# thomasjacumin/optical-flow-optimal-transport

Hardware: AMD Instinct MI355X
Metric: BB solver iters/sec on 640×480×32 grid (higher is better)
Workload: dtype f64; 1 GPU; FOTO Benamou-Brenier outer iteration, 640x480x32, r=1, eps=1e-2, CG rtol=1e-6 (scipy rule), stop rules off; cg_mode=spectral-gauss, parallelism=single GPU

## Files before the change

optical-flow-optimal-transport_amd/csrc/foto_bb.cpp:

```cpp
#include <rccl/rccl.h>

#include <algorithm>
#include <chrono>
#include <cmath>
#include <cstddef>
#include <cstring>
#include <memory>
#include <utility>

#include "foto_devmem.h"
#include "foto_internal.h"
#include "foto_spectral.h"
#include "foto_xfer.h"

namespace foto {

#define FOTO_NCCL_CHECK(call)                                                                 \
    do {                                                                                     \
        ncclResult_t r_ = (call);                                                            \
        if (r_ != ncclSuccess) {                                                             \
            ::foto::set_error("%s:%d %s: %s", __FILE__, __LINE__, #call, ncclGetErrorString(r_)); \
            return FOTO_ERR_COMM;                                                            \
        }                                                                                    \
    } while (0)
// ... 227 lines not shown
    hipStream_t user = nullptr;
};

static int load_rho(foto_bb_ctx* c, Shard& s, const RhoSrc& src) {
    const int64_t nxy = (int64_t)c->Nx * c->Ny;
    if (!src.i0) {
        FOTO_HIP_CHECK(hipMemcpyAsync(s.rho0, src.h0, nxy * sizeof(double), hipMemcpyHostToDevice, c->s));
        FOTO_HIP_CHECK(hipMemcpyAsync(s.rhoT, src.hT, nxy * sizeof(double), hipMemcpyHostToDevice, c->s));
        return 0;
    }
    if (!c->sh.empty() && c->sh[0].get() != &s) {
        FOTO_HIP_CHECK(hipMemcpyAsync(s.rho0, c->sh[0]->rho0, nxy * sizeof(double), hipMemcpyDeviceToDevice, c->s));
        FOTO_HIP_CHECK(hipMemcpyAsync(s.rhoT, c->sh[0]->rhoT, nxy * sizeof(double), hipMemcpyDeviceToDevice, c->s));
        return 0;
    }
    FOTO_TRY(c->link.enter(src.user, c->s));
    FOTO_HIP_CHECK(launch_ingest(*src.i0, c->Nx, c->Ny, s.rho0, c->s));
    FOTO_HIP_CHECK(launch_ingest(*src.iT, c->Nx, c->Ny, s.rhoT, c->s));
    if (src.normalize) {
        if (!c->nrm) {
            FOTO_TRY(s.alloc(sizeof(double) * (2 + (size_t)capped_blocks(nxy, SUM_MAX_BLOCKS)), &c->nrm));
        }
        double* const rho[2] = {s.rho0, s.rhoT};
        for (int k = 0; k < 2; ++k) {
            FOTO_HIP_CHECK(launch_sum(nxy, rho[k], c->nrm + 2, c->nrm + k, c->s));
            FOTO_HIP_CHECK(launch_div_scalar(nxy, rho[k], c->nrm + k, c->s));
        }
        FOTO_HIP_CHECK(hipMemcpyAsync(c->hsum, c->nrm, 2 * sizeof(double), hipMemcpyDeviceToHost, c->s));
    }
    return 0;
}

static int init_fields(foto_bb_ctx* c, Shard& s, const RhoSrc& src) {
    FOTO_TRY(load_rho(c, s, src));
    FOTO_HIP_CHECK(launch_init_mu(s.g, s.rho0, s.rhoT, s.mu[0], s.mu[1], s.mu[2], s.q[0], s.q[1], s.q[2], c->s));
    return 0;
}

static RhoSrc dev_src(const foto_image* f0, const foto_image* f1, int normalize, void* stream) {
    RhoSrc src;
    src.i0 = f0;
    src.iT = f1;
    src.normalize = normalize != 0;
    src.user = (hipStream_t)stream;
    return src;
}
static int dev_src_done(foto_bb_ctx* c, const RhoSrc& src, double* sums2_or_null) {
    FOTO_TRY(c->link.leave(c->s, src.user));
    if (sums2_or_null) {
        sums2_or_null[0] = src.normalize ? c->hsum[0] : 1.0;
        sums2_or_null[1] = src.normalize ? c->hsum[1] : 1.0;
    }
    return 0;
}

static int ctx_init(foto_bb_ctx* c, const RhoSrc& src) {
    const int64_t nxy = (int64_t)c->Nx * c->Ny;
    if (c->o.device >= 0) FOTO_HIP_CHECK(hipSetDevice(c->o.device));
    FOTO_TRY(stream_acquire(&c->s));
    FOTO_HIP_CHECK(hipHostMalloc((void**)&c->hS, sizeof(CGScal)));
    const int W = c->W;
    for (int k = 0; k < 2; ++k) {
        FOTO_HIP_CHECK(hipHostMalloc((void**)&c->hgath[k], sizeof(double) * 4 * W,
                                     hipHostMallocMapped | hipHostMallocCoherent));
        FOTO_HIP_CHECK(hipHostGetDevicePointer((void**)&c->dgath[k], c->hgath[k], 0));
    }
    for (auto& p : c->ph)
        for (int k = 0; k < 4; ++k)
            FOTO_HIP_CHECK(hipEventCreateWithFlags(&p[k], k < 3 ? hipEventDisableSystemFence : hipEventDefault));
    for (auto& e : c->fl) FOTO_HIP_CHECK(hipEventCreate(&e));
    if (c->rccl) {
        ncclUniqueId id;
        memcpy(&id, c->o.nccl_id, sizeof(id));
        FOTO_NCCL_CHECK(ncclCommInitRank(&c->nc, W, id, c->o.rank));
        if (c->tn.comm_stream) {
            FOTO_TRY(stream_acquire(&c->sc));
            FOTO_HIP_CHECK(hipEventCreateWithFlags(&c->cfork, hipEventDisableTiming));
            FOTO_HIP_CHECK(hipEventCreateWithFlags(&c->cjoin, hipEventDisableTiming));
            for (auto& e : c->cpart) FOTO_HIP_CHECK(hipEventCreateWithFlags(&e, hipEventDisableTiming));
        }
    }
    const int nlocal = c->rccl ? 1 : W;
    {
        c->fuse = c->tn.fuse_pr;
        c->pipe = W == 1 && c->fuse && c->o.cg_mode == 3 && c->tn.pipe;
        c->phase_force = c->tn.phase_ev;
        c->hcrit = W == 1 && c->fuse && c->tn.host_crit;
        const unsigned ff = c->hcrit ? hipEventDisableSystemFence : 0u;
        for (auto& e : c->fin) FOTO_HIP_CHECK(hipEventCreateWithFlags(&e, hipEventDisableTiming | ff));
    }
    for (int j = 0; j < nlocal; ++j) {
        auto sp = std::make_unique<Shard>();
        Shard& s = *sp;
        s.rank = c->rccl ? c->o.rank : j;
        s.g.Nt = c->Nt; s.g.Ny = c->Ny; s.g.Nx = c->Nx; s.g.nxy = nxy;
        if (split_planes(c->Nt, W, s.rank, &s.g.t0, &s.g.nloc) != 0) {
            set_error("world size %d exceeds Nt = %d (each rank needs >= 1 time slab)", W, c->Nt);
            return FOTO_ERR_ARG;
        }
        for (int f = 0; f < 3; ++f) { FOTO_TRY(s.alloc_field(&s.mu[f], c->s)); FOTO_TRY(s.alloc_field(&s.q[f], c->s)); }
        if (c->fuse)
            for (int f = 0; f < 3; ++f) FOTO_TRY(s.alloc_field(&s.nu[f], c->s));
        if (c->pipe) {
            for (int f = 0; f < 3; ++f) FOTO_TRY(s.alloc_field(&s.xi[f], c->s));
            FOTO_TRY(s.alloc_field(&s.phi_alt, c->s, 2));
        }
        if (c->fuse && W > 1) {
            FOTO_TRY(s.alloc_field(&s.wt, c->s));
            FOTO_TRY(s.alloc_zeroed(sizeof(double) * 8 * nxy, &s.edge, c->s));
        }
        FOTO_TRY(s.alloc_field(&s.phi, c->s, 2));
        FOTO_TRY(s.alloc_field(&s.rv, c->s));
        FOTO_TRY(s.alloc_field(&s.p[0], c->s));
        FOTO_TRY(s.alloc_field(&s.p[1], c->s));
        for (double** plane : {&s.rho0, &s.rhoT, &s.px, &s.py, &s.fu, &s.fv, &s.fm})
            FOTO_TRY(s.alloc(nxy * sizeof(double), plane));
        const int64_t nb = std::max<int64_t>(march_blocks(s.g), flat_blocks((int64_t)s.g.nloc * nxy));
        s.rb.cap = (int)std::max<int64_t>(2 * nb, 3 * (int64_t)prox_rhs_blocks(s.g, c->tn.pr_tch));
        FOTO_TRY(s.alloc(sizeof(double) * s.rb.cap, &s.rb.partials));
        FOTO_TRY(s.alloc_zeroed(sizeof(unsigned) * 64, &s.rb.ticket, c->s));
        FOTO_TRY(s.alloc_zeroed(sizeof(double) * 4 * W, &s.gath, c->s));
        FOTO_TRY(s.alloc_zeroed(sizeof(CGScal), &s.S, c->s));
        FOTO_TRY(init_fields(c, s, src));
        if (c->o.cg_mode >= 1 && c->o.cg_mode <= 3) {
            s.spec.reset(new SpectralPlan());
            FOTO_TRY(s.spec->init(s.g, s.rank, W, c->r, c->eps, c->o.cg_mode, c->tn, c->s));
        }
        c->sh.push_back(std::move(sp));
    }
    if (c->pipe && !(c->sh[0]->spec && c->sh[0]->spec->gauss())) c->pipe = false;
    FOTO_HIP_CHECK(hipStreamSynchronize(c->s));
    return 0;
}


static CGArgs cg_args(foto_bb_ctx* c, const Shard& s) {
    CGArgs a;
    a.r = c->r;
    a.eps = c->eps;
    a.rtol = c->o.cg_rtol;
    a.world = c->W;
    a.rank = s.rank;
    return a;
}

static int cg_iteration(foto_bb_ctx* c, int k) {
    const int W = c->W;
    const bool fused = (W == 1);
    if (!fused)
        for (auto& sp : c->sh) {
            Shard& s = *sp;
            FOTO_HIP_CHECK(launch_cg_pupd(s.g, k, s.rv, s.p[k & 1], s.p[(k + 1) & 1], s.S, s.gath_rr(), cg_args(c, s),
                                          c->s));
        }
    if (!fused) FOTO_TRY(halo(c, [k](Shard& s) { return s.p[(k + 1) & 1]; }));
    for (auto& sp : c->sh) {
        Shard& s = *sp;
        const CGArgs a = cg_args(c, s);
        const double nv = (double)s.g.nloc * (double)s.g.nxy;
        hipEvent_t e = c->kt.start(c->s);
        FOTO_HIP_CHECK(launch_cg_dir(s.g, k, s.rv, s.p[k & 1], s.p[(k + 1) & 1], a, s.S, s.rb, s.gath_rr(),
                                     s.gath_pap(W), fused ? 1 : 0, c->s));
        c->kt.stop(e, c->s, FOTO_K_CG_DIR, fused ? (k == 0 ? 16.0 : 24.0) * nv : 8.0 * nv);
    }
    FOTO_TRY(allgather(c, [W](Shard& s) { return s.gath_pap(W); }, 1));
    for (auto& sp : c->sh) {
        Shard& s = *sp;
// ... 1398 lines not shown
```

optical-flow-optimal-transport_amd/csrc/foto_internal.h:

```cpp
#pragma once

#include <hip/hip_runtime.h>

#include <algorithm>
#include <cstdint>
#include <cstdlib>
#include <cstdio>
#include <string>
#include <vector>

#include "../../include/foto.h"
#include "foto_tuning.h"

namespace foto {

void set_error(const char* fmt, ...);

#define FOTO_HIP_CHECK(call)                                                                  \
    do {                                                                                     \
        hipError_t e_ = (call);                                                              \
        if (e_ != hipSuccess) {                                                              \
            ::foto::set_error("%s:%d %s: %s", __FILE__, __LINE__, #call, hipGetErrorString(e_)); \
            return FOTO_ERR_HIP;                                                             \
        }                                                                                    \
// ... 117 lines not shown
    size_t count_before(size_t m) const {
        size_t n = 0;
        while (n < pend.size() && pend[n].id < m) ++n;
        return n;
    }
    void discard_from(size_t m) {
        const size_t keep = count_before(m);
        for (size_t k = keep; k < pend.size(); ++k) {
            pool.push_back(pend[k].a);
            pool.push_back(pend[k].b);
        }
        pend.resize(keep);
    }
    void resolve_upto(size_t m) { resolve_first(count_before(m)); }
    void resolve_first(size_t n) {
        n = std::min(n, pend.size());
        for (size_t k = 0; k < n; ++k) {
            Pend& p = pend[k];
            float t = 0.f;
            if (hipEventElapsedTime(&t, p.a, p.b) == hipSuccess) {
                this->n[p.cls] += 1;
                ms[p.cls] += t;
                bytes[p.cls] += p.bytes;
            }
            pool.push_back(p.a);
            pool.push_back(p.b);
        }
        pend.erase(pend.begin(), pend.begin() + n);
    }
    void resolve() { resolve_first(pend.size()); }
    void reset() {
        std::fill(n, n + 8, 0);
        std::fill(ms, ms + 8, 0.0);
        std::fill(bytes, bytes + 8, 0.0);
    }
    ~KTimer() {
        for (auto& p : pend) { (void)hipEventDestroy(p.a); (void)hipEventDestroy(p.b); }
        for (auto e : pool) (void)hipEventDestroy(e);
    }
};


struct CGArgs {
    double r, eps, rtol;
    int world, rank;
};

hipError_t launch_apply_A(const Geo& g, const double* p, double* out, double r, double eps, int lap_only,
                          hipStream_t s);
hipError_t launch_grad_st(const Geo& g, const double* phi, double* gt, double* gx, double* gy, hipStream_t s);
hipError_t launch_div_st(const Geo& g, const double* wt, const double* wx, const double* wy, double* out,
                         hipStream_t s);
hipError_t launch_grad2(int Nx, int Ny, const double* f, double* gx, double* gy, int bcD, hipStream_t s);
hipError_t launch_div2(int Nx, int Ny, const double* u, const double* v, double* out, int bcD, double sign,
                       hipStream_t s);
hipError_t launch_grad2_forward(int Nx, int Ny, const double* f, double* gx, double* gy, hipStream_t s);
hipError_t launch_stepB(int64_t M, const double* pa, const double* p1, const double* p2, double* qa,
                        double* q1, double* q2, hipStream_t s);
hipError_t launch_init_mu(const Geo& g, const double* rho0, const double* rhoT, double* mut, double* mux,
                          double* muy, double* qt, double* qx, double* qy, hipStream_t s);
hipError_t launch_rhs(const Geo& g, const double* mut, const double* mux, const double* muy, const double* qt,
                      const double* qx, const double* qy, const double* rho0, const double* rhoT, double r,
                      double* F, RedBuf rb, double* gath, int rank, hipStream_t s);
constexpr int REPORT_PIECE = 2048;
inline int report_pieces(int64_t nxy) { return (int)((nxy + REPORT_PIECE - 1) / REPORT_PIECE); }
struct ReportIn {
    const double *rho, *m1, *m2, *phi;
    const double *rho_lo, *rho_hi, *phi_lo, *phi_hi;
    const double *rho0, *rhoT;
};
hipError_t launch_report(const Geo& g, const ReportIn& in, double* part, unsigned* ticket, double* out,
                         hipStream_t s);
hipError_t launch_cg_dir(const Geo& g, int k, const double* rvec, const double* pold, double* pnew,
                         const CGArgs& a, CGScal* S, RedBuf rb, const double* gath_rr, double* gath_pap,
                         int fused, hipStream_t s);
hipError_t launch_cg_pupd(const Geo& g, int k, const double* rvec, const double* pold, double* pnew,
                          CGScal* S, const double* gath_rr, const CGArgs& a, hipStream_t s);
hipError_t launch_cg_upd(const Geo& g, int k, const double* p, double* x, double* rvec, const CGArgs& a,
                         CGScal* S, RedBuf rb, const double* gath_pap, double* gath_rr, hipStream_t s);
hipError_t launch_prox(const Geo& g, const double* phi, double* mut, double* mux, double* muy, double* qt,
                       double* qx, double* qy, double r, RedBuf rb, double* gath, int rank, hipStream_t s,
                       const int* guard = nullptr);
int prox_rhs_blocks(const Geo& g, int tch);
hipError_t launch_prox_rhs(const Geo& g, const double* phi, const double* mut, const double* mux, const double* muy,
                           double* nut, double* nux, double* nuy, const double* rho0, const double* rhoT, double r,
                           double* F, RedBuf rb, double* gath_crit, double* gath_rr, int tch, hipStream_t s,
                           const int* guard = nullptr, int defer_lo = 0, int defer_hi = 0, double* wt_out = nullptr,
                           double* edge = nullptr, double* hcrit = nullptr, int wt_pre = 0);
hipError_t launch_wt_pre(const Geo& g, const double* phi, const double* mut, const double* mux, const double* muy,
                         double r, double* wt, int defer_lo, int defer_hi, hipStream_t s, const int* guard = nullptr);
hipError_t launch_rhs_edge(const Geo& g, int n, const double* wt, const double* edge, const double* rho0,
                           const double* rhoT, double r, double* F, RedBuf rb, double* gath_rr, hipStream_t s,
                           const int* guard = nullptr);
hipError_t launch_q_from_phi(const Geo& g, const double* phi, const double* mut, const double* mux,
                             const double* muy, double* qt, double* qx, double* qy, double r, hipStream_t s);
hipError_t launch_traj(const Geo& g, const double* phi, int n_lo, int n_hi, double* px, double* py,
                       int init, hipStream_t s);
hipError_t launch_flow_record(int Nx, int Ny, const double* px, const double* py, void* ou, void* ov, void* om,
                              int dtype, int layout, hipStream_t s);

hipError_t launch_track(const Geo& g, const double* phi, int n_lo, int n_hi, const void* pts, int pts_dtype,
                        const double* pos_in, double* pos_out, void* out, int dtype, int64_t M, int all_steps,
                        hipStream_t s);

hipError_t launch_dot_self(int64_t n, const double* x, RedBuf rb, double* gath, int rank, hipStream_t s);

hipError_t launch_gn_coeffs(int w, int h, const double* f1, const double* f2, double* fx, double* fy,
                            double* ft, hipStream_t s);
hipError_t launch_gn_rhs(int w, int h, const double* fx, const double* fy, const double* f2, const double* ft,
                         double* b, hipStream_t s);
hipError_t launch_gn_apply(int w, int h, const double* fx, const double* fy, const double* f2, double alpha,
                           double lam, const double* x, double* y, hipStream_t s);
int gn_bj_solve(const double* f1, const double* f2, int w, int h, double alpha, double lam, double rtol, int maxiter,
                double* u, double* v, double* m, int* iterations);

int image_check(const foto_image* im, int w, int h, const char* who);
int image_dev_check(const foto_image* im, int w, int h, int device, const char* who);
int dev_ptr_check(const void* p, size_t bytes, int device, const char* who, const char* what);
int export_check(const void* out, int dtype, int layout, int64_t n, int device, const char* who);
int track_arg_check(const void* pts, const void* out, int64_t M, int all_steps, const char* who);
int track_dtype_check(const void* p, int dtype, const char* who, const char* what);
hipError_t launch_ingest(const foto_image& im, int w, int h, double* dst, hipStream_t s);
hipError_t launch_sum(int64_t n, const double* x, double* part, double* tot, hipStream_t s);
hipError_t launch_div_scalar(int64_t n, double* x, const double* S, hipStream_t s);
hipError_t launch_export(int64_t n, const double* a, const double* b, const double* c, void* out, int dtype,
                         int layout, hipStream_t s);
constexpr int FRAMES_MAX = 128;
struct FrameArgs {
    const double* a[FRAMES_MAX];
    const double* b[FRAMES_MAX];
    double w[FRAMES_MAX];
};
hipError_t launch_frames(const FrameArgs& fa, int count, int64_t n, double scale, void* out, int dtype,
                         hipStream_t s);

constexpr int MAPS_MAX = 128;
constexpr int MT_W = 32, MT_H = 8;
constexpr int PLANE_SEGS = 32;
struct MapTimes {
    double s[MAPS_MAX];
};
struct PlaneSegs {
    const double* base[PLANE_SEGS];
    int t0[PLANE_SEGS], nloc[PLANE_SEGS];
    int n;
};
hipError_t launch_plane_table(const PlaneSegs& sg, int64_t nxy, const double** table, hipStream_t s);
hipError_t launch_maps(const double* const* table, int Nt, int Nx, int Ny, const double* s, int count, int inv_iters,
                       void* out, int dtype, hipStream_t st);
hipError_t launch_interp(const double* const* table, int Nt, int Nx, int Ny, const foto_image& f0, int64_t sc0,
                         const foto_image& f1, int64_t sc1, int channels, const double* s, int count, int inv_iters,
                         void* out, int out_dtype, hipStream_t st);
int maps_arg_check(const double* s, const void* out, int count, int inv_iters, int Nt, const char* who);
int interp_frame_check(const foto_image* f, int channels, int64_t stride_c, int w, int h, const char* who);
size_t interp_frame_bytes(const foto_image* f, int channels, int64_t stride_c, int w, int h);
int flow_check(const foto_flow* fl, int w, int h, const char* who);
size_t flow_bytes(const foto_flow* fl, int w, int h);
inline bool overlaps(const void* a, size_t na, const void* b, size_t nb) {
    const uintptr_t a0 = (uintptr_t)a, b0 = (uintptr_t)b;
    return a0 < b0 + nb && b0 < a0 + na;
}

struct DevScratch {
    void* p = nullptr;
    size_t cap = 0;
    int reserve(size_t bytes, hipStream_t s) {
// ... 20 lines not shown
```

optical-flow-optimal-transport_amd/csrc/foto_kernels.hip:

```cpp
#include "foto_devutil.h"
#include "foto_internal.h"
#include "foto_reduce.h"

namespace foto {


__device__ __forceinline__ double row_A(const Geo& g, int t, int y, int x, double c, double xm, double xp,
                                        double ym, double yp, double tm, double tp, double r, double reps) {
    const bool ht = t > 0, hT = t < g.Nt - 1, hy = y > 0, hY = y < g.Ny - 1, hx = x > 0, hX = x < g.Nx - 1;
    const double cnt = (double)((int)ht + (int)hT + (int)hy + (int)hY + (int)hx + (int)hX);
    const double mr = -r;
    const double dg = r * cnt + reps;
    double s = 0.0;
    if (ht) s += mr * tm;
    if (hy) s += mr * ym;
    if (hx) s += mr * xm;
    s += dg * c;
    if (hX) s += mr * xp;
    if (hY) s += mr * yp;
    if (hT) s += mr * tp;
    return s;
}

__device__ __forceinline__ double row_L(const Geo& g, int t, int y, int x, double c, double xm, double xp,
                                        double ym, double yp, double tm, double tp) {
    const bool ht = t > 0, hT = t < g.Nt - 1, hy = y > 0, hY = y < g.Ny - 1, hx = x > 0, hX = x < g.Nx - 1;
    const double cnt = (double)((int)ht + (int)hT + (int)hy + (int)hY + (int)hx + (int)hX);
    double s = 0.0;
    if (ht) s += tm;
    if (hy) s += ym;
    if (hx) s += xm;
    s += (-cnt) * c;
    if (hX) s += xp;
    if (hY) s += yp;
    if (hT) s += tp;
    return s;
}

__device__ __forceinline__ int xcd_tile(int b) {
    constexpr int NXCD = 8;
    const int nb = gridDim.x, per = nb / NXCD, rem = nb % NXCD;
    const int xcd = b % NXCD, local = b / NXCD;
    return xcd * per + min(xcd, rem) + local;
}

template <class Val, class Body>
__device__ __forceinline__ void march(const Geo& g, int tile_blk, Val val, Body body) {
    const int tile = xcd_tile(tile_blk);
    constexpr int LW = TX + 2, LP = (TY + 2) * LW;
    __shared__ double lds[2 * LP];
    const int ntx = (g.Nx + TX - 1) / TX;
    const int x0 = (tile % ntx) * TX, y0 = (tile / ntx) * TY;
    const int tid = threadIdx.x, tx = tid & (TX - 1), ty = tid / TX;
    const int x = x0 + tx, y = y0 + ty;
    const bool in = (x < g.Nx) && (y < g.Ny);
    const int64_t off = in ? (int64_t)y * g.Nx + x : 0;
    int hx = -1, hy = -1, hl = -1;
    if (tid < TX) { hx = x0 + tid; hy = y0 - 1; hl = tid + 1; }
    else if (tid < 2 * TX) { hx = x0 + tid - TX; hy = y0 + TY; hl = (TY + 1) * LW + (tid - TX) + 1; }
    else if (tid < 2 * TX + TY) { hx = x0 - 1; hy = y0 + (tid - 2 * TX); hl = (tid - 2 * TX + 1) * LW; }
    else if (tid < 2 * TX + 2 * TY) { hx = x0 + TX; hy = y0 + (tid - 2 * TX - TY); hl = (tid - 2 * TX - TY + 1) * LW + TX + 1; }
    const bool hv = hl >= 0 && hx >= 0 && hx < g.Nx && hy >= 0 && hy < g.Ny;
    const int64_t hoff = hv ? (int64_t)hy * g.Nx + hx : 0;
    const int ci = (ty + 1) * LW + tx + 1;
    const bool has_lo = g.t0 > 0, has_hi = g.t0 + g.nloc < g.Nt;

    double cm = 0.0, cc = 0.0, cn = 0.0, hc = 0.0;
    if (in) {
        if (has_lo) cm = val(-1, off);
        cc = val(0, off);
        if (g.nloc > 1 || has_hi) cn = val(1, off);
    }
    if (hv) hc = val(0, hoff);
    for (int l = 0; l < g.nloc; ++l) {
        double* buf = lds + (l & 1) * LP;
        buf[ci] = cc;
        if (hl >= 0) buf[hl] = hc;
        double cnn = 0.0, hnn = 0.0;
        if (in && (l + 2 < g.nloc || (l + 2 == g.nloc && has_hi))) cnn = val(l + 2, off);
        if (hv && l + 1 < g.nloc) hnn = val(l + 1, hoff);
        __syncthreads();
        if (in) {
// ... 464 lines not shown
    double a, b, c;
    project_K(pa[i], p1[i], p2[i], a, b, c);
    qa[i] = a;
    q1[i] = b;
    q2[i] = c;
}

hipError_t launch_stepB(int64_t M, const double* pa, const double* p1, const double* p2, double* qa, double* q1,
                        double* q2, hipStream_t s) {
    k_stepB<<<flat_blocks(M), NT, 0, s>>>(M, pa, p1, p2, qa, q1, q2);
    return hipGetLastError();
}


__global__ __launch_bounds__(NT) void k_prox(Geo g, const double* __restrict__ phi, double* __restrict__ mut,
                                             double* __restrict__ mux, double* __restrict__ muy,
                                             double* __restrict__ qt, double* __restrict__ qx,
                                             double* __restrict__ qy, double r, double inv_r, RedBuf rb,
                                             double* gath, int rank, const int* __restrict__ guard) {
    if (guard && *guard == 0) return;
    const int64_t nxy = g.nxy;
    double num = 0.0, den = 0.0;
    march(g, blockIdx.x, [&](int l, int64_t off) { return phi[l * nxy + off]; },
          [&](int l, int t, int64_t off, int x, int y, double c, double xm, double xp, double ym, double yp,
              double tm, double tp) {
              const int64_t i = l * nxy + off;
              const double gt = d1w(t, g.Nt, tm, c, tp);
              const double gx = d1w(x, g.Nx, xm, c, xp);
              const double gy = d1w(y, g.Ny, ym, c, yp);
              const double m0 = mut[i], m1 = mux[i], m2 = muy[i];
              double a, b1, b2;
              project_K(gt + inv_r * m0, gx + inv_r * m1, gy + inv_r * m2, a, b1, b2);
              qt[i] = a;
              qx[i] = b1;
              qy[i] = b2;
              double n0 = m0 + r * (gt - a);
              n0 = (n0 < 0.0) ? 0.0 : n0;
              mut[i] = n0;
              mux[i] = m1 + r * (gx - b1);
              muy[i] = m2 + r * (gy - b2);
              const double gg = gx * gx + gy * gy;
              num += n0 * fabs(gt + 0.5 * gg);
              den += n0 * gg;
          });
    double v[2] = {num, den}, tot[2];
    if (grid_reduce_last<2>(v, rb, tot) && threadIdx.x == 0) {
        gath[2 * rank] = tot[0];
        gath[2 * rank + 1] = tot[1];
    }
}

hipError_t launch_prox(const Geo& g, const double* phi, double* mut, double* mux, double* muy, double* qt,
                       double* qx, double* qy, double r, RedBuf rb, double* gath, int rank, hipStream_t s,
                       const int* guard) {
    k_prox<<<march_blocks(g), NT, 0, s>>>(g, phi, mut, mux, muy, qt, qx, qy, r, 1.0 / r, rb, gath, rank, guard);
    return hipGetLastError();
}

__global__ __launch_bounds__(NT) void k_q_from_phi(Geo g, const double* __restrict__ phi,
                                                   const double* __restrict__ mut, const double* __restrict__ mux,
                                                   const double* __restrict__ muy, double* __restrict__ qt,
                                                   double* __restrict__ qx, double* __restrict__ qy, double inv_r) {
    const int64_t nxy = g.nxy;
    march(g, blockIdx.x, [&](int l, int64_t off) { return phi[l * nxy + off]; },
          [&](int l, int t, int64_t off, int x, int y, double c, double xm, double xp, double ym, double yp,
              double tm, double tp) {
              const int64_t i = l * nxy + off;
              double a, b1, b2;
              project_K(d1w(t, g.Nt, tm, c, tp) + inv_r * mut[i], d1w(x, g.Nx, xm, c, xp) + inv_r * mux[i],
                        d1w(y, g.Ny, ym, c, yp) + inv_r * muy[i], a, b1, b2);
              qt[i] = a;
              qx[i] = b1;
              qy[i] = b2;
          });
}

hipError_t launch_q_from_phi(const Geo& g, const double* phi, const double* mut, const double* mux,
                             const double* muy, double* qt, double* qx, double* qy, double r, hipStream_t s) {
    k_q_from_phi<<<march_blocks(g), NT, 0, s>>>(g, phi, mut, mux, muy, qt, qx, qy, 1.0 / r);
    return hipGetLastError();
}

constexpr int PR_X = 64, PR_Y = 8;
constexpr int PR_VPT = 1;
constexpr int PR_NT = PR_X * PR_Y / PR_VPT;
constexpr int PR_YV = PR_Y / PR_VPT;
constexpr int PR_PW = PR_X + 2, PR_PH = PR_Y + 2;
constexpr int PR_FW = PR_X + 4, PR_FH = PR_Y + 4;
constexpr int PR_HALO = 2 * PR_PW + 2 * PR_Y;
constexpr int PR_FN = PR_FW * PR_FH;
constexpr int PR_FR = (PR_FN + PR_NT - 1) / PR_NT;
static_assert(PR_X == 64 && PR_NT <= 1024 && PR_HALO <= PR_NT && PR_Y % PR_VPT == 0,
              "whole rows per thread, ring voxels on the first threads");
constexpr int PR_WPE = 4;

template <bool EDGE, bool INTERIOR>
__device__ __forceinline__ void prox_rhs_body(
        Geo g, const double* __restrict__ phi, const double* __restrict__ mut, const double* __restrict__ mux,
        const double* __restrict__ muy, double* __restrict__ nut, double* __restrict__ nux, double* __restrict__ nuy,
        const double* __restrict__ rho0, const double* __restrict__ rhoT, double r, double inv_r,
        double* __restrict__ F, int tch, int defer_lo, int defer_hi, double* __restrict__ wt_out,
        double* __restrict__ edge, int wt_pre, double (*fr)[PR_FN], double (*wb)[2][PR_PH * PR_PW], int ch, int x0,
        int y0, double& num_out, double& den_out, double& ff_out) {
    const int Nt = g.Nt, Nx = g.Nx, Ny = g.Ny, t0 = g.t0;
    const int64_t nxy = g.nxy;
    const int l0 = ch * tch, l1 = min(g.nloc, l0 + tch);
    const int tid = threadIdx.x;
    const int opx = 1 + (tid & (PR_X - 1));
    const int ox = x0 - 1 + opx;
    int opy[PR_VPT], oy[PR_VPT], ooff[PR_VPT];
    bool own[PR_VPT];
#pragma unroll
    for (int v = 0; v < PR_VPT; ++v) {
        opy[v] = 1 + tid / PR_X + v * PR_YV;
        oy[v] = y0 - 1 + opy[v];
        own[v] = INTERIOR || (ox < Nx && oy[v] < Ny);
        ooff[v] = own[v] ? oy[v] * Nx + ox : 0;
    }
    int hpx = 0, hpy = 0;
    if (tid < PR_PW) { hpx = tid; hpy = 0; }
    else if (tid < 2 * PR_PW) { hpx = tid - PR_PW; hpy = PR_PH - 1; }
    else if (tid < 2 * PR_PW + PR_Y) { hpx = 0; hpy = 1 + tid - 2 * PR_PW; }
    else { hpx = PR_PW - 1; hpy = 1 + tid - 2 * PR_PW - PR_Y; }
    const int hx = x0 - 1 + hpx, hy = y0 - 1 + hpy;
    const bool hal = tid < PR_HALO && (INTERIOR || (hx >= 0 && hx < Nx && hy >= 0 && hy < Ny));
    const int hoff = hal ? hy * Nx + hx : 0;
    int foff[PR_FR];
    bool fin[PR_FR];
#pragma unroll
    for (int j = 0; j < PR_FR; ++j) {
        const int idx = tid + j * PR_NT;
        const int fy = idx / PR_FW, fx = idx - fy * PR_FW;
        const int xx = x0 - 2 + fx, yy = y0 - 2 + fy;
        fin[j] = idx < PR_FN && (INTERIOR || (xx >= 0 && xx < Nx && yy >= 0 && yy < Ny));
        foff[j] = fin[j] ? yy * Nx + xx : 0;
    }
    if (!EDGE) defer_lo = defer_hi = 0;
    const int pa = max(l0 - 1, defer_lo ? 0 : -t0), pz = min(l1, defer_hi ? g.nloc - 1 : Nt - 1 - t0);
    const int nl = g.nloc;
    double fv[PR_FR];
    auto load_phi_to = [&](int p, double (&v)[PR_FR]) {
        const bool ok = t0 + p >= 0 && p <= pz + 1 && t0 + p < Nt;
#pragma unroll
        for (int j = 0; j < PR_FR; ++j)
            v[j] = (ok && fin[j]) ? phi[p * nxy + foff[j]] : 0.0;
    };
    auto store_phi_from = [&](int p, const double (&v)[PR_FR]) {
#pragma unroll
        for (int j = 0; j < PR_FR; ++j)
            if (tid + j * PR_NT < PR_FN) fr[p & 3][tid + j * PR_NT] = v[j];
    };
    auto load_phi = [&](int p) { load_phi_to(p, fv); };
    auto store_phi = [&](int p) { store_phi_from(p, fv); };
    double om[PR_VPT][3], hm[3] = {0.0, 0.0, 0.0};
#pragma unroll
    for (int v = 0; v < PR_VPT; ++v) om[v][0] = om[v][1] = om[v][2] = 0.0;
    auto load_mu = [&](int p) {
        if (p > pz) return;
#pragma unroll
        for (int v = 0; v < PR_VPT; ++v) {
            if (own[v]) {
                om[v][0] = __builtin_nontemporal_load(&mut[p * nxy + ooff[v]]);
                om[v][1] = __builtin_nontemporal_load(&mux[p * nxy + ooff[v]]);
                om[v][2] = __builtin_nontemporal_load(&muy[p * nxy + ooff[v]]);
            }
        }
        if (hal) {
            hm[0] = __builtin_nontemporal_load(&mut[p * nxy + hoff]);
            hm[1] = __builtin_nontemporal_load(&mux[p * nxy + hoff]);
            hm[2] = __builtin_nontemporal_load(&muy[p * nxy + hoff]);
        }
    };
    auto stepb = [&](int p, int px, int py, int xg, int yg, const double (&m)[3], double (&w)[3], double& n0o,
                     double& ao, double& gto, double& gxo, double& gyo, double (&nu)[3]) {
        const int t = t0 + p;
        const int fi = (py + 1) * PR_FW + px + 1;
        const double* P = fr[p & 3];
        const double c = P[fi];
        const double tm = t > 0 ? fr[(p - 1) & 3][fi] : 0.0, tp = t < Nt - 1 ? fr[(p + 1) & 3][fi] : 0.0;
        const double gt = d1w(t, Nt, tm, c, tp);
        const double gx = d1w(xg, Nx, P[fi - 1], c, P[fi + 1]);
        const double gy = d1w(yg, Ny, P[fi - PR_FW], c, P[fi + PR_FW]);
        double a, b1, b2;
        project_K(gt + inv_r * m[0], gx + inv_r * m[1], gy + inv_r * m[2], a, b1, b2);
        double n0 = m[0] + r * (gt - a);
        n0 = (n0 < 0.0) ? 0.0 : n0;
        nu[0] = n0;
        nu[1] = m[1] + r * (gx - b1);
        nu[2] = m[2] + r * (gy - b2);
        w[0] = nu[0] - r * a;
        w[1] = nu[1] - r * b1;
        w[2] = nu[2] - r * b2;
        n0o = n0;
        ao = a;
        gto = gt;
        gxo = gx;
        gyo = gy;
    };
    double num = 0.0, den = 0.0, ff = 0.0;
    double wtm[PR_VPT], wtc[PR_VPT], wtn[PR_VPT], bcm[PR_VPT], bcq[PR_VPT], bcm_n[PR_VPT], bcq_n[PR_VPT];
#pragma unroll
    for (int v = 0; v < PR_VPT; ++v) wtm[v] = wtc[v] = wtn[v] = bcm[v] = bcq[v] = bcm_n[v] = bcq_n[v] = 0.0;
    auto plane = [&](int p, const double (&mo)[PR_VPT][3], const double (&mh)[3]) {
        const bool mine = p >= l0 && p < l1;
#pragma unroll
        for (int v = 0; v < PR_VPT; ++v) {
            if (own[v]) {
                double w[3], nu[3], n0, a, gt, gx, gy;
                stepb(p, opx, opy[v], ox, oy[v], mo[v], w, n0, a, gt, gx, gy, nu);
                if (mine) {
                    const int64_t i = p * nxy + ooff[v];
                    __builtin_nontemporal_store(nu[0], &nut[i]);
                    __builtin_nontemporal_store(nu[1], &nux[i]);
                    __builtin_nontemporal_store(nu[2], &nuy[i]);
                    const double gg = gx * gx + gy * gy;
                    num += n0 * fabs(gt + 0.5 * gg);
                    den += n0 * gg;
                }
                wb[p & 1][0][opy[v] * PR_PW + opx] = w[1];
                wb[p & 1][1][opy[v] * PR_PW + opx] = w[2];
                wtn[v] = w[0];
                bcm_n[v] = n0;
                bcq_n[v] = a;
            }
        }
        if (hal) {
            double w[3], nu[3], n0, a, gt, gx, gy;
            stepb(p, hpx, hpy, hx, hy, mh, w, n0, a, gt, gx, gy, nu);
            wb[p & 1][0][hpy * PR_PW + hpx] = w[1];
            wb[p & 1][1][hpy * PR_PW + hpx] = w[2];
        }
    };
    {
        double f0[PR_FR], f1[PR_FR], f2[PR_FR];
        load_phi_to(pa - 1, f0);
        load_phi_to(pa, f1);
        load_phi_to(pa + 1, f2);
        load_phi(pa + 2);
        load_mu(pa);
        store_phi_from(pa - 1, f0);
        store_phi_from(pa, f1);
        store_phi_from(pa + 1, f2);
    }
    __syncthreads();
    for (int p = pa; p <= l1; ++p) {
        store_phi(p + 2);
        load_phi(p + 3);
        double cm[PR_VPT][3];
#pragma unroll
        for (int v = 0; v < PR_VPT; ++v) { cm[v][0] = om[v][0]; cm[v][1] = om[v][1]; cm[v][2] = om[v][2]; }
        const double chm[3] = {hm[0], hm[1], hm[2]};
        load_mu(p + 1);
        if (p <= pz) plane(p, cm, chm);
        else {
#pragma unroll
            for (int v = 0; v < PR_VPT; ++v) wtn[v] = 0.0;
        }
        const int n = p - 1, tn = t0 + n;
        const bool deferred = (defer_lo && n == 0) || (defer_hi && n == nl - 1);
#pragma unroll
        for (int v = 0; v < PR_VPT; ++v) {
            if (EDGE && own[v] && n >= l0) {
                if (((defer_lo && n <= 1) || (defer_hi && n >= nl - 2)) && !(wt_pre && deferred))
                    wt_out[n * nxy + ooff[v]] = wtc[v];
                if (deferred) {
                    const int ci = opy[v] * PR_PW + opx;
                    double* E = edge + ooff[v] + ((defer_lo && n == 0) ? 0 : 4 * nxy);
                    E[0] = wb[n & 1][0][ci];
                    E[nxy] = wb[n & 1][1][ci];
                    E[2 * nxy] = bcm[v];
                    E[3 * nxy] = bcq[v];
                    if (defer_lo && defer_hi && nl == 1) {
                        E[4 * nxy] = E[0];
                        E[5 * nxy] = E[nxy];
                        E[6 * nxy] = bcm[v];
                        E[7 * nxy] = bcq[v];
                    }
                }
            }
            if (own[v] && n >= l0 && !deferred) {
                const double* WX = wb[n & 1][0];
                const double* WY = wb[n & 1][1];
                const int ci = opy[v] * PR_PW + opx;
                const int oo = ooff[v], yv = oy[v];
                double s = 0.0;
                acc_d1w(s, tn, Nt, wtm[v], wtc[v], wtn[v]);
                acc_d1w(s, ox, Nx, (INTERIOR || ox > 0) ? WX[ci - 1] : 0.0, WX[ci],
                        (INTERIOR || ox < Nx - 1) ? WX[ci + 1] : 0.0);
                acc_d1w(s, yv, Ny, (INTERIOR || yv > 0) ? WY[ci - PR_PW] : 0.0, WY[ci],
                        (INTERIOR || yv < Ny - 1) ? WY[ci + PR_PW] : 0.0);
                if (tn == 0) s -= (rho0[oo] - bcm[v]) + r * bcq[v];
                if (tn == Nt - 1) s += (rhoT[oo] - bcm[v]) + r * bcq[v];
                F[n * nxy + oo] = s;
                ff += s * s;
            }
            wtm[v] = wtc[v];
            wtc[v] = wtn[v];
            bcm[v] = bcm_n[v];
            bcq[v] = bcq_n[v];
        }
        __syncthreads();
    }
    num_out = num;
    den_out = den;
    ff_out = ff;
}

template <bool EDGE>
__global__ __launch_bounds__(PR_NT) __attribute__((amdgpu_waves_per_eu(PR_WPE))) void k_prox_rhs(
        Geo g, const double* __restrict__ phi, const double* __restrict__ mut, const double* __restrict__ mux,
        const double* __restrict__ muy, double* __restrict__ nut, double* __restrict__ nux, double* __restrict__ nuy,
        const double* __restrict__ rho0, const double* __restrict__ rhoT, double r, double inv_r,
        double* __restrict__ F, RedBuf rb, double* gath_crit, double* gath_rr, const int* __restrict__ guard, int tch,
        int defer_lo, int defer_hi, double* __restrict__ wt_out, double* __restrict__ edge, double* hcrit,
        int wt_pre) {
    if (guard && *guard == 0) return;
    __shared__ double fr[4][PR_FN];
    __shared__ double wb[2][2][PR_PH * PR_PW];
    const int Nx = g.Nx, Ny = g.Ny;
    const int ntx = (Nx + PR_X - 1) / PR_X, ntiles = ntx * ((Ny + PR_Y - 1) / PR_Y);
    const int lin = xcd_tile(blockIdx.x);
    const int ch = lin / ntiles, tile = lin - ch * ntiles;
    const int x0 = (tile % ntx) * PR_X, y0 = (tile / ntx) * PR_Y;
    double num, den, ff;
    if (x0 >= 2 && x0 + PR_X + 2 <= Nx && y0 >= 2 && y0 + PR_Y + 2 <= Ny)
        prox_rhs_body<EDGE, true>(g, phi, mut, mux, muy, nut, nux, nuy, rho0, rhoT, r, inv_r, F, tch, defer_lo,
                                  defer_hi, wt_out, edge, wt_pre, fr, wb, ch, x0, y0, num, den, ff);
    else
        prox_rhs_body<EDGE, false>(g, phi, mut, mux, muy, nut, nux, nuy, rho0, rhoT, r, inv_r, F, tch, defer_lo,
                                   defer_hi, wt_out, edge, wt_pre, fr, wb, ch, x0, y0, num, den, ff);
    double v[3] = {num, den, ff}, tot[3];
    if (grid_reduce_last<3, PR_NT>(v, rb, tot) && threadIdx.x == 0) {
        gath_crit[0] = tot[0];
        gath_crit[1] = tot[1];
        if (gath_rr) gath_rr[0] = tot[2];
        if (hcrit) {
            hcrit[0] = tot[0];
            hcrit[1] = tot[1];
            __threadfence_system();
        }
    }
}

static int prox_rhs_tch(const Geo& g, int tch) { return std::min(tch, g.nloc); }

int prox_rhs_blocks(const Geo& g, int tch) {
    tch = prox_rhs_tch(g, tch);
    return ((g.Nx + PR_X - 1) / PR_X) * ((g.Ny + PR_Y - 1) / PR_Y) * ((g.nloc + tch - 1) / tch);
}

hipError_t launch_prox_rhs(const Geo& g, const double* phi, const double* mut, const double* mux, const double* muy,
                           double* nut, double* nux, double* nuy, const double* rho0, const double* rhoT, double r,
                           double* F, RedBuf rb, double* gath_crit, double* gath_rr, int tch, hipStream_t s,
                           const int* guard, int defer_lo, int defer_hi, double* wt_out, double* edge, double* hcrit,
                           int wt_pre) {
    const int nb = prox_rhs_blocks(g, tch);
    if (rb.cap < 3 * nb) return hipErrorInvalidValue;
    if ((defer_lo || defer_hi) && (!wt_out || !edge)) return hipErrorInvalidValue;
    if (defer_lo || defer_hi)
        k_prox_rhs<true><<<nb, PR_NT, 0, s>>>(g, phi, mut, mux, muy, nut, nux, nuy, rho0, rhoT, r, 1.0 / r, F, rb,
                                              gath_crit, gath_rr, guard, prox_rhs_tch(g, tch), defer_lo, defer_hi, wt_out, edge,
                                              hcrit, wt_pre);
    else
        k_prox_rhs<false><<<nb, PR_NT, 0, s>>>(g, phi, mut, mux, muy, nut, nux, nuy, rho0, rhoT, r, 1.0 / r, F, rb,
                                               gath_crit, gath_rr, guard, prox_rhs_tch(g, tch), 0, 0, nullptr, nullptr,
                                               hcrit, 0);
    return hipGetLastError();
}

__global__ __launch_bounds__(NT) void k_wt_pre(Geo g, int pa, int pb, const double* __restrict__ phi,
                                               const double* __restrict__ mut, const double* __restrict__ mux,
                                               const double* __restrict__ muy, double r, double inv_r,
                                               double* __restrict__ wt, const int* __restrict__ guard) {
    if (guard && *guard == 0) return;
    const int64_t nxy = g.nxy;
    const int64_t off = (int64_t)blockIdx.x * NT + threadIdx.x;
    if (off >= nxy) return;
    const int p = blockIdx.y == 0 ? pa : pb;
    const int y = (int)(off / g.Nx), x = (int)(off - (int64_t)y * g.Nx), t = g.t0 + p;
    const int64_t i = (int64_t)p * nxy + off;
    const double c = phi[i];
    const double tm = t > 0 ? phi[i - nxy] : 0.0, tp = t < g.Nt - 1 ? phi[i + nxy] : 0.0;
    const double gt = d1w(t, g.Nt, tm, c, tp);
    const double gx = d1w(x, g.Nx, x > 0 ? phi[i - 1] : 0.0, c, x < g.Nx - 1 ? phi[i + 1] : 0.0);
    const double gy = d1w(y, g.Ny, y > 0 ? phi[i - g.Nx] : 0.0, c, y < g.Ny - 1 ? phi[i + g.Nx] : 0.0);
    const double m0 = mut[i], m1 = mux[i], m2 = muy[i];
    double a, b1, b2;
    project_K(gt + inv_r * m0, gx + inv_r * m1, gy + inv_r * m2, a, b1, b2);
    double n0 = m0 + r * (gt - a);
    n0 = (n0 < 0.0) ? 0.0 : n0;
    wt[i] = n0 - r * a;
}

hipError_t launch_wt_pre(const Geo& g, const double* phi, const double* mut, const double* mux, const double* muy,
                         double r, double* wt, int defer_lo, int defer_hi, hipStream_t s, const int* guard) {
    if (!defer_lo && !defer_hi) return hipSuccess;
    const int pa = defer_lo ? 0 : g.nloc - 1, pb = g.nloc - 1;
    const int np = (defer_lo && defer_hi && g.nloc > 1) ? 2 : 1;
    k_wt_pre<<<dim3((unsigned)flat_blocks(g.nxy), np), NT, 0, s>>>(g, pa, pb, phi, mut, mux, muy, r, 1.0 / r, wt,
                                                                  guard);
    return hipGetLastError();
}

__global__ __launch_bounds__(NT) void k_rhs_edge(Geo g, int n, const double* __restrict__ wt,
                                                 const double* __restrict__ E, const double* __restrict__ rho0,
                                                 const double* __restrict__ rhoT, double r, double* __restrict__ F,
                                                 RedBuf rb, double* gath_rr, const int* __restrict__ guard) {
    if (guard && *guard == 0) return;
    const int64_t nxy = g.nxy;
    const int64_t off = (int64_t)blockIdx.x * NT + threadIdx.x;
    double ff = 0.0;
    if (off < nxy) {
        const int y = (int)(off / g.Nx), x = (int)(off - (int64_t)y * g.Nx), tn = g.t0 + n;
        const double* WX = E;
        const double* WY = E + nxy;
        const int64_t i = (int64_t)n * nxy + off;
        double s = 0.0;
        acc_d1w(s, tn, g.Nt, wt[i - nxy], wt[i], wt[i + nxy]);
        acc_d1w(s, x, g.Nx, x > 0 ? WX[off - 1] : 0.0, WX[off], x < g.Nx - 1 ? WX[off + 1] : 0.0);
        acc_d1w(s, y, g.Ny, y > 0 ? WY[off - g.Nx] : 0.0, WY[off], y < g.Ny - 1 ? WY[off + g.Nx] : 0.0);
        const double bcm = E[2 * nxy + off], bcq = E[3 * nxy + off];
        if (tn == 0) s -= (rho0[off] - bcm) + r * bcq;
        if (tn == g.Nt - 1) s += (rhoT[off] - bcm) + r * bcq;
        F[i] = s;
        ff = s * s;
    }
    if (!gath_rr) return;
    double v[1] = {ff}, tot[1];
    if (grid_reduce_last<1>(v, rb, tot) && threadIdx.x == 0) gath_rr[0] += tot[0];
}

hipError_t launch_rhs_edge(const Geo& g, int n, const double* wt, const double* edge, const double* rho0,
                           const double* rhoT, double r, double* F, RedBuf rb, double* gath_rr, hipStream_t s,
                           const int* guard) {
    if (n < 0 || n >= g.nloc) return hipErrorInvalidValue;
    k_rhs_edge<<<flat_blocks(g.nxy), NT, 0, s>>>(g, n, wt, edge, rho0, rhoT, r, F, rb, gath_rr, guard);
    return hipGetLastError();
}


// ... 195 lines not shown
```

Baseline: 1866 iters/s.

## Specialize steady-state planes in fused prox-rhs kernel with uniform base addressing

Restructures the fused prox/RHS time-marching loop into boundary and steady-state phases. Steady-state planes are a compile-time specialization that drops the time-boundary checks and boundary-condition bookkeeping, and that part of the loop is unrolled by two with ping-pong mu registers. Addresses are rebuilt as a wave-uniform 64-bit plane base (readfirstlane) plus a 32-bit per-lane byte offset. The aim is to cut VGPR pressure and per-load 64-bit address arithmetic. It adds a size guard that disables fusion when the offsets could overflow 32 bits, plus more code complexity and more kernel code.

```diff
diff --git a/optical-flow-optimal-transport_amd/csrc/foto_bb.cpp b/optical-flow-optimal-transport_amd/csrc/foto_bb.cpp
--- a/optical-flow-optimal-transport_amd/csrc/foto_bb.cpp
+++ b/optical-flow-optimal-transport_amd/csrc/foto_bb.cpp
@@ -333,7 +333,9 @@
     }
     const int nlocal = c->rccl ? 1 : W;
     {
-        c->fuse = c->tn.fuse_pr;
+        Geo plane{};
+        plane.Nx = c->Nx;
+        c->fuse = c->tn.fuse_pr && prox_rhs_fits(plane);
         c->pipe = W == 1 && c->fuse && c->o.cg_mode == 3 && c->tn.pipe;
         c->phase_force = c->tn.phase_ev;
         c->hcrit = W == 1 && c->fuse && c->tn.host_crit;
diff --git a/optical-flow-optimal-transport_amd/csrc/foto_internal.h b/optical-flow-optimal-transport_amd/csrc/foto_internal.h
--- a/optical-flow-optimal-transport_amd/csrc/foto_internal.h
+++ b/optical-flow-optimal-transport_amd/csrc/foto_internal.h
@@ -223,6 +223,7 @@
                        double* qx, double* qy, double r, RedBuf rb, double* gath, int rank, hipStream_t s,
                        const int* guard = nullptr);
 int prox_rhs_blocks(const Geo& g, int tch);
+bool prox_rhs_fits(const Geo& g);
 hipError_t launch_prox_rhs(const Geo& g, const double* phi, const double* mut, const double* mux, const double* muy,
                            double* nut, double* nux, double* nuy, const double* rho0, const double* rhoT, double r,
                            double* F, RedBuf rb, double* gath_crit, double* gath_rr, int tch, hipStream_t s,
diff --git a/optical-flow-optimal-transport_amd/csrc/foto_kernels.hip b/optical-flow-optimal-transport_amd/csrc/foto_kernels.hip
--- a/optical-flow-optimal-transport_amd/csrc/foto_kernels.hip
+++ b/optical-flow-optimal-transport_amd/csrc/foto_kernels.hip
@@ -1,3 +1,5 @@
+#include <type_traits>
+
 #include "foto_devutil.h"
 #include "foto_internal.h"
 #include "foto_reduce.h"
@@ -628,6 +630,20 @@
 }
 
 constexpr int PR_X = 64, PR_Y = 8;
+
+template <class T>
+__device__ __forceinline__ T* byte_at(T* base, uint32_t off) {
+    return (T*)((const char*)base + off);
+}
+__device__ __forceinline__ uint32_t in_loop(uint32_t off) {
+    asm volatile("" : "+v"(off));
+    return off;
+}
+__device__ __forceinline__ int64_t uniform64(int64_t v) {
+    const uint32_t lo = __builtin_amdgcn_readfirstlane((uint32_t)v);
+    const uint32_t hi = __builtin_amdgcn_readfirstlane((uint32_t)((uint64_t)v >> 32));
+    return (int64_t)(((uint64_t)hi << 32) | lo);
+}
 constexpr int PR_VPT = 1;
 constexpr int PR_NT = PR_X * PR_Y / PR_VPT;
 constexpr int PR_YV = PR_Y / PR_VPT;
@@ -652,9 +668,11 @@
     const int64_t nxy = g.nxy;
     const int l0 = ch * tch, l1 = min(g.nloc, l0 + tch);
     const int tid = threadIdx.x;
+    const int64_t org = (int64_t)(y0 - 2) * Nx + (x0 - 2);
     const int opx = 1 + (tid & (PR_X - 1));
     const int ox = x0 - 1 + opx;
     int opy[PR_VPT], oy[PR_VPT], ooff[PR_VPT];
+    uint32_t oob[PR_VPT];
     bool own[PR_VPT];
 #pragma unroll
     for (int v = 0; v < PR_VPT; ++v) {
@@ -662,6 +680,7 @@
         oy[v] = y0 - 1 + opy[v];
         own[v] = INTERIOR || (ox < Nx && oy[v] < Ny);
         ooff[v] = own[v] ? oy[v] * Nx + ox : 0;
+        oob[v] = own[v] ? 8u * (uint32_t)((opy[v] + 1) * Nx + opx + 1) : 0u;
     }
     int hpx = 0, hpy = 0;
     if (tid < PR_PW) { hpx = tid; hpy = 0; }
@@ -670,8 +689,8 @@
     else { hpx = PR_PW - 1; hpy = 1 + tid - 2 * PR_PW - PR_Y; }
     const int hx = x0 - 1 + hpx, hy = y0 - 1 + hpy;
     const bool hal = tid < PR_HALO && (INTERIOR || (hx >= 0 && hx < Nx && hy >= 0 && hy < Ny));
-    const int hoff = hal ? hy * Nx + hx : 0;
-    int foff[PR_FR];
+    const uint32_t hob = hal ? 8u * (uint32_t)((hpy + 1) * Nx + hpx + 1) : 0u;
+    uint32_t fob[PR_FR];
     bool fin[PR_FR];
 #pragma unroll
     for (int j = 0; j < PR_FR; ++j) {
@@ -679,52 +698,66 @@
         const int fy = idx / PR_FW, fx = idx - fy * PR_FW;
         const int xx = x0 - 2 + fx, yy = y0 - 2 + fy;
         fin[j] = idx < PR_FN && (INTERIOR || (xx >= 0 && xx < Nx && yy >= 0 && yy < Ny));
-        foff[j] = fin[j] ? yy * Nx + xx : 0;
+        fob[j] = fin[j] ? 8u * (uint32_t)(fy * Nx + fx) : 0u;
     }
     if (!EDGE) defer_lo = defer_hi = 0;
     const int pa = max(l0 - 1, defer_lo ? 0 : -t0), pz = min(l1, defer_hi ? g.nloc - 1 : Nt - 1 - t0);
     const int nl = g.nloc;
+    const int ps = max(l0 + 1, 2 - t0), pe = EDGE ? ps - 1 : min(pz - 2, Nt - 4 - t0);
     double fv[PR_FR];
-    auto load_phi_to = [&](int p, double (&v)[PR_FR]) {
-        const bool ok = t0 + p >= 0 && p <= pz + 1 && t0 + p < Nt;
+    auto load_phi_to = [&](auto st, int p, double (&v)[PR_FR]) {
+        constexpr bool ST = decltype(st)::value;
+        const bool ok = ST || (t0 + p >= 0 && p <= pz + 1 && t0 + p < Nt);
+        const int64_t pb = uniform64(p * nxy + org);
 #pragma unroll
         for (int j = 0; j < PR_FR; ++j)
-            v[j] = (ok && fin[j]) ? phi[p * nxy + foff[j]] : 0.0;
+            v[j] = (ok && fin[j]) ? *byte_at(phi + pb, in_loop(fob[j])) : 0.0;
     };
     auto store_phi_from = [&](int p, const double (&v)[PR_FR]) {
 #pragma unroll
         for (int j = 0; j < PR_FR; ++j)
             if (tid + j * PR_NT < PR_FN) fr[p & 3][tid + j * PR_NT] = v[j];
     };
-    auto load_phi = [&](int p) { load_phi_to(p, fv); };
     auto store_phi = [&](int p) { store_phi_from(p, fv); };
-    double om[PR_VPT][3], hm[3] = {0.0, 0.0, 0.0};
-#pragma unroll
-    for (int v = 0; v < PR_VPT; ++v) om[v][0] = om[v][1] = om[v][2] = 0.0;
-    auto load_mu = [&](int p) {
-        if (p > pz) return;
+    auto load_mu = [&](auto st, int p, double (&mo)[PR_VPT][3], double (&mh)[3]) {
+        constexpr bool ST = decltype(st)::value;
+        if (!ST && p > pz) return;
+        const int64_t pb = uniform64(p * nxy + org);
+        if (hal && (ST || (p >= l0 && p < l1))) {
+            const uint32_t o = in_loop(hob);
+            mh[0] = __builtin_nontemporal_load(byte_at(mut + pb, o));
+            mh[1] = __builtin_nontemporal_load(byte_at(mux + pb, o));
+            mh[2] = __builtin_nontemporal_load(byte_at(muy + pb, o));
+        }
 #pragma unroll
         for (int v = 0; v < PR_VPT; ++v) {
             if (own[v]) {
-                om[v][0] = __builtin_nontemporal_load(&mut[p * nxy + ooff[v]]);
-                om[v][1] = __builtin_nontemporal_load(&mux[p * nxy + ooff[v]]);
-                om[v][2] = __builtin_nontemporal_load(&muy[p * nxy + ooff[v]]);
+                const uint32_t o = in_loop(oob[v]);
+                mo[v][0] = __builtin_nontemporal_load(byte_at(mut + pb, o));
+                mo[v][1] = __builtin_nontemporal_load(byte_at(mux + pb, o));
+                mo[v][2] = __builtin_nontemporal_load(byte_at(muy + pb, o));
             }
         }
-        if (hal) {
-            hm[0] = __builtin_nontemporal_load(&mut[p * nxy + hoff]);
-            hm[1] = __builtin_nontemporal_load(&mux[p * nxy + hoff]);
-            hm[2] = __builtin_nontemporal_load(&muy[p * nxy + hoff]);
-        }
     };
-    auto stepb = [&](int p, int px, int py, int xg, int yg, const double (&m)[3], double (&w)[3], double& n0o,
-                     double& ao, double& gto, double& gxo, double& gyo, double (&nu)[3]) {
+    auto load_rho = [&](int n, double (&rc)[PR_VPT]) {
+        const int tn = t0 + n;
+        if (n < l0) return;
+#pragma unroll
+        for (int v = 0; v < PR_VPT; ++v) {
+            if (own[v] && tn == 0) rc[v] = *byte_at(rho0 + org, in_loop(oob[v]));
+            if (own[v] && tn == Nt - 1) rc[v] = *byte_at(rhoT + org, in_loop(oob[v]));
+        }
+    };
+    auto stepb = [&](auto st, int p, int px, int py, int xg, int yg, const double (&m)[3], double (&w)[3],
+                     double& n0o, double& ao, double& gto, double& gxo, double& gyo, double (&nu)[3]) {
+        constexpr bool ST = decltype(st)::value;
         const int t = t0 + p;
         const int fi = (py + 1) * PR_FW + px + 1;
         const double* P = fr[p & 3];
         const double c = P[fi];
-        const double tm = t > 0 ? fr[(p - 1) & 3][fi] : 0.0, tp = t < Nt - 1 ? fr[(p + 1) & 3][fi] : 0.0;
-        const double gt = d1w(t, Nt, tm, c, tp);
+        const double tm = (ST || t > 0) ? fr[(p - 1) & 3][fi] : 0.0;
+        const double tp = (ST || t < Nt - 1) ? fr[(p + 1) & 3][fi] : 0.0;
+        const double gt = ST ? 0.5 * (tp - tm) : d1w(t, Nt, tm, c, tp);
         const double gx = d1w(xg, Nx, P[fi - 1], c, P[fi + 1]);
         const double gy = d1w(yg, Ny, P[fi - PR_FW], c, P[fi + PR_FW]);
         double a, b1, b2;
@@ -747,57 +780,51 @@
     double wtm[PR_VPT], wtc[PR_VPT], wtn[PR_VPT], bcm[PR_VPT], bcq[PR_VPT], bcm_n[PR_VPT], bcq_n[PR_VPT];
 #pragma unroll
     for (int v = 0; v < PR_VPT; ++v) wtm[v] = wtc[v] = wtn[v] = bcm[v] = bcq[v] = bcm_n[v] = bcq_n[v] = 0.0;
-    auto plane = [&](int p, const double (&mo)[PR_VPT][3], const double (&mh)[3]) {
-        const bool mine = p >= l0 && p < l1;
+    auto plane = [&](auto st, int p, const double (&mo)[PR_VPT][3], const double (&mh)[3]) {
+        constexpr bool ST = decltype(st)::value;
+        const bool mine = ST || (p >= l0 && p < l1);
 #pragma unroll
         for (int v = 0; v < PR_VPT; ++v) {
             if (own[v]) {
                 double w[3], nu[3], n0, a, gt, gx, gy;
-                stepb(p, opx, opy[v], ox, oy[v], mo[v], w, n0, a, gt, gx, gy, nu);
+                stepb(st, p, opx, opy[v], ox, oy[v], mo[v], w, n0, a, gt, gx, gy, nu);
                 if (mine) {
-                    const int64_t i = p * nxy + ooff[v];
-                    __builtin_nontemporal_store(nu[0], &nut[i]);
-                    __builtin_nontemporal_store(nu[1], &nux[i]);
-                    __builtin_nontemporal_store(nu[2], &nuy[i]);
+                    const uint32_t o = in_loop(oob[v]);
+                    const int64_t pb = uniform64(p * nxy + org);
+                    __builtin_nontemporal_store(nu[0], byte_at(nut + pb, o));
+                    __builtin_nontemporal_store(nu[1], byte_at(nux + pb, o));
+                    __builtin_nontemporal_store(nu[2], byte_at(nuy + pb, o));
                     const double gg = gx * gx + gy * gy;
                     num += n0 * fabs(gt + 0.5 * gg);
                     den += n0 * gg;
+                    wb[p & 1][0][opy[v] * PR_PW + opx] = w[1];
+                    wb[p & 1][1][opy[v] * PR_PW + opx] = w[2];
                 }
-                wb[p & 1][0][opy[v] * PR_PW + opx] = w[1];
-                wb[p & 1][1][opy[v] * PR_PW + opx] = w[2];
                 wtn[v] = w[0];
-                bcm_n[v] = n0;
-                bcq_n[v] = a;
+                if (!ST) {
+                    bcm_n[v] = n0;
+                    bcq_n[v] = a;
+                }
             }
         }
-        if (hal) {
+        if (hal && mine) {
             double w[3], nu[3], n0, a, gt, gx, gy;
-            stepb(p, hpx, hpy, hx, hy, mh, w, n0, a, gt, gx, gy, nu);
+            stepb(st, p, hpx, hpy, hx, hy, mh, w, n0, a, gt, gx, gy, nu);
             wb[p & 1][0][hpy * PR_PW + hpx] = w[1];
             wb[p & 1][1][hpy * PR_PW + hpx] = w[2];
         }
     };
-    {
-        double f0[PR_FR], f1[PR_FR], f2[PR_FR];
-        load_phi_to(pa - 1, f0);
-        load_phi_to(pa, f1);
-        load_phi_to(pa + 1, f2);
-        load_phi(pa + 2);
-        load_mu(pa);
-        store_phi_from(pa - 1, f0);
-        store_phi_from(pa, f1);
-        store_phi_from(pa + 1, f2);
-    }
-    __syncthreads();
-    for (int p = pa; p <= l1; ++p) {
+    auto step = [&](auto st, int p, const double (&mc)[PR_VPT][3], const double (&hc)[3], double (&mn)[PR_VPT][3],
+                    double (&hn)[3]) {
+        constexpr bool ST = decltype(st)::value;
+        double rc[PR_VPT];
+#pragma unroll
+        for (int v = 0; v < PR_VPT; ++v) rc[v] = 0.0;
+        if (!ST) load_rho(p - 1, rc);
         store_phi(p + 2);
-        load_phi(p + 3);
-        double cm[PR_VPT][3];
-#pragma unroll
-        for (int v = 0; v < PR_VPT; ++v) { cm[v][0] = om[v][0]; cm[v][1] = om[v][1]; cm[v][2] = om[v][2]; }
-        const double chm[3] = {hm[0], hm[1], hm[2]};
-        load_mu(p + 1);
-        if (p <= pz) plane(p, cm, chm);
+        load_phi_to(st, p + 3, fv);
+        load_mu(st, p + 1, mn, hn);
+        if (ST || p <= pz) plane(st, p, mc, hc);
         else {
 #pragma unroll
             for (int v = 0; v < PR_VPT; ++v) wtn[v] = 0.0;
@@ -824,28 +851,87 @@
                     }
                 }
             }
-            if (own[v] && n >= l0 && !deferred) {
+            if (own[v] && (ST || n >= l0) && !deferred) {
                 const double* WX = wb[n & 1][0];
                 const double* WY = wb[n & 1][1];
                 const int ci = opy[v] * PR_PW + opx;
-                const int oo = ooff[v], yv = oy[v];
+                const int yv = oy[v];
                 double s = 0.0;
-                acc_d1w(s, tn, Nt, wtm[v], wtc[v], wtn[v]);
+                if (ST) {
+                    s += -0.5 * wtm[v];
+                    s += 0.5 * wtn[v];
+                } else {
+                    acc_d1w(s, tn, Nt, wtm[v], wtc[v], wtn[v]);
+                }
                 acc_d1w(s, ox, Nx, (INTERIOR || ox > 0) ? WX[ci - 1] : 0.0, WX[ci],
                         (INTERIOR || ox < Nx - 1) ? WX[ci + 1] : 0.0);
                 acc_d1w(s, yv, Ny, (INTERIOR || yv > 0) ? WY[ci - PR_PW] : 0.0, WY[ci],
                         (INTERIOR || yv < Ny - 1) ? WY[ci + PR_PW] : 0.0);
-                if (tn == 0) s -= (rho0[oo] - bcm[v]) + r * bcq[v];
-                if (tn == Nt - 1) s += (rhoT[oo] - bcm[v]) + r * bcq[v];
-                F[n * nxy + oo] = s;
+                if (!ST && tn == 0) s -= (rc[v] - bcm[v]) + r * bcq[v];
+                if (!ST && tn == Nt - 1) s += (rc[v] - bcm[v]) + r * bcq[v];
+                *byte_at(F + uniform64(n * nxy + org), in_loop(oob[v])) = s;
                 ff += s * s;
             }
             wtm[v] = wtc[v];
             wtc[v] = wtn[v];
-            bcm[v] = bcm_n[v];
-            bcq[v] = bcq_n[v];
+            if (!ST) {
+                bcm[v] = bcm_n[v];
+                bcq[v] = bcq_n[v];
+            }
         }
         __syncthreads();
+    };
+    double mA[PR_VPT][3], hA[3] = {0.0, 0.0, 0.0}, mB[PR_VPT][3], hB[3] = {0.0, 0.0, 0.0};
+#pragma unroll
+    for (int v = 0; v < PR_VPT; ++v) mA[v][0] = mA[v][1] = mA[v][2] = mB[v][0] = mB[v][1] = mB[v][2] = 0.0;
+    const std::false_type any_plane{};
+    const std::true_type steady{};
+    {
+        double f0[PR_FR], f1[PR_FR], f2[PR_FR];
+        load_phi_to(any_plane, pa - 1, f0);
+        load_phi_to(any_plane, pa, f1);
+        load_phi_to(any_plane, pa + 1, f2);
+        load_phi_to(any_plane, pa + 2, fv);
+        load_mu(any_plane, pa, mA, hA);
+        store_phi_from(pa - 1, f0);
+        store_phi_from(pa, f1);
+        store_phi_from(pa + 1, f2);
+    }
+    __syncthreads();
+    int p = pa;
+#pragma nounroll
+    for (int part = 0; part < 2; ++part) {
+        const int last = part == 0 ? min(ps - 1, l1) : l1;
+        for (; p <= last; ++p) {
+            double cm[PR_VPT][3];
+#pragma unroll
+            for (int v = 0; v < PR_VPT; ++v) {
+                cm[v][0] = mA[v][0];
+                cm[v][1] = mA[v][1];
+                cm[v][2] = mA[v][2];
+            }
+            const double chm[3] = {hA[0], hA[1], hA[2]};
+            step(any_plane, p, cm, chm, mA, hA);
+        }
+        if constexpr (!EDGE) {
+            if (part == 0 && p <= pe) {
+                step(steady, p, mA, hA, mB, hB);
+                for (++p; p + 1 <= pe; p += 2) {
+                    step(steady, p, mB, hB, mA, hA);
+                    step(steady, p + 1, mA, hA, mB, hB);
+                }
+#pragma unroll
+                for (int v = 0; v < PR_VPT; ++v) {
+                    mA[v][0] = mB[v][0];
+                    mA[v][1] = mB[v][1];
+                    mA[v][2] = mB[v][2];
+                    bcm[v] = bcq[v] = bcm_n[v] = bcq_n[v] = 0.0;
+                }
+                hA[0] = hB[0];
+                hA[1] = hB[1];
+                hA[2] = hB[2];
+            }
+        }
     }
     num_out = num;
     den_out = den;
@@ -895,6 +981,8 @@
     return ((g.Nx + PR_X - 1) / PR_X) * ((g.Ny + PR_Y - 1) / PR_Y) * ((g.nloc + tch - 1) / tch);
 }
 
+bool prox_rhs_fits(const Geo& g) { return 8 * ((int64_t)PR_FH * g.Nx + PR_FW) <= (int64_t)UINT32_MAX; }
+
 hipError_t launch_prox_rhs(const Geo& g, const double* phi, const double* mut, const double* mux, const double* muy,
                            double* nut, double* nux, double* nuy, const double* rho0, const double* rhoT, double r,
                            double* F, RedBuf rb, double* gath_crit, double* gath_rr, int tch, hipStream_t s,
@@ -902,6 +990,7 @@
                            int wt_pre) {
     const int nb = prox_rhs_blocks(g, tch);
     if (rb.cap < 3 * nb) return hipErrorInvalidValue;
+    if (!prox_rhs_fits(g)) return hipErrorInvalidValue;
     if ((defer_lo || defer_hi) && (!wt_out || !edge)) return hipErrorInvalidValue;
     if (defer_lo || defer_hi)
         k_prox_rhs<true><<<nb, PR_NT, 0, s>>>(g, phi, mut, mux, muy, nut, nux, nuy, rho0, rhoT, r, 1.0 / r, F, rb,
```

Result: faster. 1889 iters/s, median of 6 (+1.2%).
